# barlettacarmen/CrCNN

Hardware: AMD Instinct MI355X
Metric: encrypted images/sec (higher is better)
Workload: dtype u64

## Files before the change

### crcnn_amd/csrc/kernels_mfma.hip

```cpp
#include "kernels.h"
#include "limbred.h"
#include <algorithm>
#include <cstdlib>

typedef int v4i __attribute__((ext_vector_type(4)));
typedef int v16i __attribute__((ext_vector_type(16)));
typedef signed char i8;

#define NPL 7
#define TILE_B (NPL * 64 * 32)

struct MfmaArgs {
    const i8 *xl; const i8 *wl; u64 *ys; const ModParams *mods; const u64 *bias;
    int xcdmap;
    int mfast;
    i8 *xl_out; int lp2; unsigned zdp_out;
    int n, k, B, zdp, npos, yd, xs, ystr, yf, yo, P, F, Fp, zblks, ksteps, M, mtiles, ntiles;
    unsigned img_bytes; unsigned long long wslot_bytes; int ksteps_real;
    int flat, S, zdc; unsigned fplane;
    int sc_B;
    int acc0[8][13];
    u64 qinv[8];
};

__device__ __forceinline__ void limb_digits(u64 r, u64 q, int (&d)[NPL])
{
    long long v = r > (q >> 1) ? (long long)r - (long long)q : (long long)r;
#pragma unroll
    for (int l = 0; l < NPL; l++) { d[l] = (int)(signed char)(v & 0xff); v = (v - d[l]) >> 8; }
}

template <int NST>
__global__ void __launch_bounds__(256) __attribute__((amdgpu_waves_per_eu(1, 1))) mfma_mac_kernel(MfmaArgs a)
{
    extern __shared__ __attribute__((aligned(16))) i8 lds[];
    const int lane = threadIdx.x & 63, wave = __builtin_amdgcn_readfirstlane(threadIdx.x >> 6), wm = wave >> 1, wn = wave & 1;
    const int slots = a.n * a.k, per = a.mtiles * a.ntiles;
    int g = blockIdx.x, slot, tile;
    if ((slots & 7) == 0) { const int xcd = g & 7, r = g >> 3; slot = xcd * (slots >> 3) + r / per; tile = r % per; }
    else { slot = g / per; tile = g % per; }
    const int mt = a.mfast ? tile % a.mtiles : tile / a.ntiles, nt = a.mfast ? tile / a.mtiles : tile % a.ntiles;
    const int i = slot / a.n, s = slot % a.n;
    const int m0 = mt * 64, f0 = nt * 64;
    const ModParams m = a.mods[i];
    const u64 qinv = a.qinv[i];
    const i8 *xs = a.xl + (size_t)slot * a.B * a.img_bytes;
    const i8 *ws = a.wl + (size_t)slot * a.wslot_bytes + (size_t)f0 * 32;
    u32 src_off[7];
#pragma unroll
    for (int j = 0; j < 7; j++) {
        const int pc = wave + 4 * j;
        if (pc < 14) {
            const int c16 = pc * 64 + lane;
            const int plane = c16 >> 7, row = (c16 >> 1) & 63, half = c16 & 1;
            const int mm = min(m0 + row, a.M - 1);
            const int b = mm / (2 * a.P), p = (mm >> 1) % a.P, c = mm & 1;
            const int ox = p / a.yo, oy = p % a.yo;
            src_off[j] = a.npos == 1 ? (u32)(plane * a.zblks * (2 * a.B) + mm) * 32 + half * 16
                       : a.flat ? (u32)b * a.img_bytes + (u32)(plane * a.fplane + (c * a.npos + (ox * a.xs) * a.yd + oy * a.ystr) * a.zdc + half * 16)
                                : (u32)b * a.img_bytes + (u32)(plane * (a.npos * 2 * a.zdp) + (((ox * a.xs) * a.yd + oy * a.ystr) * 2 + c) * a.zdp + half * 16);
        } else src_off[j] = (u32)(((pc - 14) >> 1) * (a.Fp * 32) + ((pc - 14) & 1) * 1024 + lane * 16);
    }
    const int kreal = a.ksteps_real;
    auto issue = [&](int ks) {
        const int ka = min(ks, kreal - 1);
        const int tap = ka / a.zblks, zb = ka - tap * a.zblks;
        const int kx = tap / a.yf, ky = tap - kx * a.yf;
        const int fkx = ka / a.S;
        const u32 delta = a.npos == 1 ? (u32)zb * (2 * a.B) * 32 : a.flat ? (u32)(fkx * a.yd * a.zdc + (ka - fkx * a.S) * 32) : (u32)((kx * a.yd + ky) * 2 * a.zdp + zb * 32);
        i8 *dst = lds + (ks % NST) * (2 * TILE_B);
        const i8 *wt = ws + (size_t)ks * (NPL * a.Fp * 32);
#pragma unroll
        for (int j = 0; j < 7; j++) {
            const int pc = wave + 4 * j;
            const i8 *src = pc < 14 ? xs + src_off[j] + delta : wt + src_off[j];
            __builtin_amdgcn_global_load_lds((const __attribute__((address_space(1))) void *)src, (__attribute__((address_space(3))) void *)(dst + pc * 1024), 16, 0, 0);
        }
    };
    v4i acc[2][2][13];
#pragma unroll
    for (int rs = 0; rs < 2; rs++)
#pragma unroll
        for (int cs = 0; cs < 2; cs++)
#pragma unroll
            for (int d = 0; d < 13; d++) { const int b0 = a.acc0[i][d]; acc[rs][cs][d] = v4i{b0, b0, b0, b0}; }
    const int K = a.ksteps;
#pragma unroll
    for (int j = 0; j < NST - 2; j++) if (j < K) issue(j);
    const int kg = lane >> 4, r16 = lane & 15;
    const int fragA = (wm * 32 + r16) * 32 + (kg & 1) * 16, fragW = (wn * 32 + r16) * 32 + (kg & 1) * 16;
    for (int ks = 0; ks < K; ks += 2) {
        const int younger = min(NST - 4, K - 2 - ks);
        if (younger >= 1) __builtin_amdgcn_s_waitcnt(7 | (7 << 4) | (15 << 8));
        else __builtin_amdgcn_s_waitcnt(0 | (7 << 4) | (15 << 8));
        __syncthreads();
        __builtin_amdgcn_sched_barrier(0);
        if (ks + NST - 2 < K) { issue(ks + NST - 2); __builtin_amdgcn_sched_barrier(0); if (ks + NST - 1 < K) issue(ks + NST - 1); }
        __builtin_amdgcn_sched_barrier(0);
        const i8 *tA = lds + ((ks + (kg >> 1)) % NST) * (2 * TILE_B), *tW = tA + TILE_B;
        v4i w[2][NPL], av[2 * NPL];
        auto read_a = [&](int gi) { return *reinterpret_cast<const v4i *>(tA + (gi % NPL) * (64 * 32) + fragA + (gi / NPL) * (16 * 32)); };
#pragma unroll
        for (int cs = 0; cs < 2; cs++)
#pragma unroll
            for (int l = 0; l < NPL; l++) w[cs][l] = *reinterpret_cast<const v4i *>(tW + l * (64 * 32) + fragW + cs * (16 * 32));
        av[0] = read_a(0); av[1] = read_a(1);
        __builtin_amdgcn_sched_barrier(0);
#pragma unroll
        for (int gi = 0; gi < 2 * NPL; gi++) {
            const int rs = gi / NPL, l = gi % NPL;
#pragma unroll
            for (int cs = 0; cs < 2; cs++)
#pragma unroll
                for (int mm = 0; mm < NPL; mm++)
                    acc[rs][cs][l + mm] = __builtin_amdgcn_mfma_i32_16x16x64_i8(av[gi], w[cs][mm], acc[rs][cs][l + mm], 0, 0, 0);
            if (gi + 2 < 2 * NPL) av[gi + 2] = read_a(gi + 2);
            __builtin_amdgcn_sched_barrier(0);
        }
    }
    u64 *yslot = a.ys + (size_t)slot * a.B * a.F * (2 * a.P);
    const u32 P2 = 2 * a.P;
    const u32 RL = 64 * a.P;
    if (a.xl_out) __syncthreads();
#pragma unroll
    for (int rs = 0; rs < 2; rs++) {
        const u32 mbase = m0 + wm * 32 + rs * 16 + 4 * kg, bb = mbase / P2, rem = mbase - bb * P2;
#pragma unroll
        for (int cs = 0; cs < 2; cs++) {
            const int fl = wn * 32 + cs * 16 + r16, f = f0 + fl;
            const u64 bv = (a.bias && f < a.F) ? a.bias[((size_t)f * a.k + i) * a.n + s] : 0;
#pragma unroll
            for (int reg = 0; reg < 4; reg++) {
                int D[13];
#pragma unroll
                for (int d = 0; d < 13; d++) D[d] = acc[rs][cs][d][reg];
                u64 v = diag_reduce_w(D, m, qinv);
                if ((reg & 1) == 0) v = addmod(v, bv, m.q);
                if (a.xl_out) {
                    const u32 rt = wm * 32 + rs * 16 + 4 * kg + reg, bl = rt >> a.lp2, qq = rt & (P2 - 1);
                    const u64 dg = f < a.F ? balanced_digit_bytes(v, m.q) : 0;
                    i8 *sp = lds + (size_t)bl * (NPL * 2 * RL) + (qq & 1) * RL + fl * a.P + (qq >> 1);
#pragma unroll
                    for (int l = 0; l < NPL; l++) sp[(size_t)l * (2 * RL)] = (i8)(dg >> (8 * l));
                } else {
                    const u32 r = rem + reg, b = bb + (r >= P2) + (r >= 2 * P2);
                    if (mbase + reg < (u32)a.M && f < a.F) yslot[b * (u32)(a.F - 1) * P2 + (u32)f * P2 + mbase + reg] = v;
                }
                __builtin_amdgcn_sched_barrier(0);
            }
        }
    }
    if (a.xl_out) {
        __syncthreads();
        const u32 imgs = 64 >> a.lp2, b0 = (u32)m0 >> a.lp2, per_run = RL / 16, pieces = imgs * NPL * 2 * per_run;
        const u32 ch0 = (u32)f0 * a.P;
        for (u32 o = threadIdx.x; o < pieces; o += 256) {
            const u32 run = o / per_run, off = (o - run * per_run) * 16, bl = run / (NPL * 2), lc = run - bl * (NPL * 2);
            const u32 ch = ch0 + off;
            if (b0 + bl < (u32)a.B && ch < a.zdp_out)
                *reinterpret_cast<uint4 *>(a.xl_out + (size_t)slot * ((size_t)NPL * 2 * a.B * a.zdp_out)
                                           + ((size_t)((lc >> 1) * (a.zdp_out / 32) + (ch >> 5)) * (2 * a.B) + (b0 + bl) * 2 + (lc & 1)) * 32 + (ch & 31)) =
                    *reinterpret_cast<const uint4 *>(lds + (size_t)run * RL + off);
        }
    }
}

#define TILE_A (NPL * 64 * 32)
template <int NST, int MODE, bool SC = false>
__global__ void __launch_bounds__(256) __attribute__((amdgpu_waves_per_eu(2, 2))) mfma_mac2w_kernel(MfmaArgs a)
{
    extern __shared__ __attribute__((aligned(16))) i8 lds[];
    const int lane = threadIdx.x & 63, wave = __builtin_amdgcn_readfirstlane(threadIdx.x >> 6), wm = wave >> 1, wn = wave & 1;
    const int slots = a.n * a.k;
    const int fast = !SC && a.xcdmap ? (int)(blockIdx.x >> 3) : (int)blockIdx.x, slow = (int)blockIdx.y;
    const int slot = !SC && a.xcdmap ? (int)(blockIdx.x & 7) * (slots >> 3) + (int)blockIdx.z : (int)blockIdx.z;
    const int mt = SC || a.mfast ? fast : slow, nt = SC || a.mfast ? slow : fast;
    const int lgn = __builtin_ctz(a.n), i = SC ? slot : slot >> lgn, s = SC ? 0 : slot & (a.n - 1);
    const int m0 = mt * 64, f0 = nt * 32;
    if (f0 >= a.F) return;
    const ModParams m = a.mods[i];
    const u64 qinv = a.qinv[i];
    const i8 *xs = a.xl + (size_t)slot * a.B * a.img_bytes;
    const int kg = lane >> 4, r16 = lane & 15;
    const i8 *wlane = a.wl + (size_t)slot * a.wslot_bytes + (size_t)(f0 + wn * 16 + r16) * 32 + (kg & 1) * 16 + (size_t)(kg >> 1) * (NPL * a.Fp * 32);
    const int wplane = a.Fp * 32, wstep = NPL * a.Fp * 32;
    u32 src_off[4]; int pcs[4];
    {
        const int row = ((wave & 1) << 5) + (lane >> 1), half = lane & 1;
        const int mm = min(m0 + row, a.M - 1);
        const int b = mm / (2 * a.P), rem = mm - b * (2 * a.P), p = rem >> 1, c = rem & 1;
        const int ox = p / a.yo, oy = p - ox * a.yo;
        const u32 rowpart = MODE == 0 ? (u32)mm * 32 + half * 16
                          : MODE == 1 ? (u32)b * a.img_bytes + (u32)((c * a.npos + (ox * a.xs) * a.yd + oy * a.ystr) * a.zdc + half * 16)
                                   : (u32)b * a.img_bytes + (u32)((((ox * a.xs) * a.yd + oy * a.ystr) * 2 + c) * a.zdp + half * 16);
        const u32 pstride = MODE == 0 ? (u32)(a.zblks * (2 * a.B)) * 32 : MODE == 1 ? a.fplane : (u32)(a.npos * 2 * a.zdp);
#pragma unroll
        for (int j = 0; j < 4; j++) {
            pcs[j] = wave + 4 * j < 14 ? wave + 4 * j : wave + 8;
            src_off[j] = rowpart + (u32)(pcs[j] >> 1) * pstride;
        }
    }
    const int kreal = a.ksteps_real;
    int iss = 0, ibuf = 0, zb = 0, ky = 0, kx = 0;
    u32 delta = 0;
    auto issue_a = [&](int ks) {
        (void)ks;
        i8 *dst = lds + ibuf * TILE_A;
#pragma unroll
        for (int j = 0; j < 4; j++)
            __builtin_amdgcn_global_load_lds((const __attribute__((address_space(1))) void *)(xs + src_off[j] + delta), (__attribute__((address_space(3))) void *)(dst + pcs[j] * 1024), 16, 0, 0);
        iss++; ibuf = ibuf + 1 == NST ? 0 : ibuf + 1;
        if (iss < kreal) {
            if (MODE == 0) delta += (u32)(2 * a.B) * 32;
            else if (MODE == 1) { if (++zb == a.S) { zb = 0; kx++; } delta = (u32)(kx * a.yd * a.zdc + zb * 32); }
            else { if (++zb == a.zblks) { zb = 0; if (++ky == a.yf) { ky = 0; kx++; } } delta = (u32)((kx * a.yd + ky) * 2 * a.zdp + zb * 32); }
        }
    };
    auto load_w = [&](int ks, v4i (&w)[NPL]) {
        const i8 *pw = wlane + (size_t)ks * wstep;
#pragma unroll
        for (int l = 0; l < NPL; l++) w[l] = *reinterpret_cast<const v4i *>(pw + (size_t)l * wplane);
    };
    v4i acc[2][13];
#pragma unroll
    for (int rs = 0; rs < 2; rs++)
#pragma unroll
        for (int d = 0; d < 13; d++) { const int b0 = a.acc0[i][d]; acc[rs][d] = v4i{b0, b0, b0, b0}; }
    const int K = a.ksteps;
    const int fragA = (wm * 32 + r16) * 32 + (kg & 1) * 16;
    auto dstep = [&](int ks, v4i (&wuse)[NPL], v4i (&wload)[NPL]) {
        if (ks + 2 < K) __builtin_amdgcn_s_waitcnt(11 | (7 << 4) | (15 << 8));
        else __builtin_amdgcn_s_waitcnt(0 | (7 << 4) | (15 << 8));
        __syncthreads();
        __builtin_amdgcn_sched_barrier(0);
        if (ks + 3 < K) issue_a(ks + 3);
        __builtin_amdgcn_sched_barrier(0);
        if (ks + 4 < K) { load_w(ks + 4, wload); __builtin_amdgcn_sched_barrier(0); issue_a(ks + 4); }
        __builtin_amdgcn_sched_barrier(0);
        const i8 *tA = lds + ((ks + (kg >> 1)) % NST) * TILE_A;
        v4i av[2 * NPL];
        auto read_a = [&](int gi) { return *reinterpret_cast<const v4i *>(tA + (gi % NPL) * (64 * 32) + fragA + (gi / NPL) * (16 * 32)); };
        av[0] = read_a(0); av[1] = read_a(1); av[2] = read_a(2);
        __builtin_amdgcn_sched_barrier(0);
#pragma unroll
        for (int gi = 0; gi < 2 * NPL; gi++) {
            const int rs = gi / NPL, l = gi % NPL;
#pragma unroll
            for (int mm = 0; mm < NPL; mm++)
                acc[rs][l + mm] = __builtin_amdgcn_mfma_i32_16x16x64_i8(av[gi], wuse[mm], acc[rs][l + mm], 0, 0, 0);
            if (gi + 3 < 2 * NPL) av[gi + 3] = read_a(gi + 3);
            __builtin_amdgcn_sched_barrier(0);
        }
    };
    v4i w0[NPL], w1[NPL], w2[NPL];
    issue_a(0); if (1 < K) issue_a(1);
    __builtin_amdgcn_sched_barrier(0);
    load_w(0, w0);
    __builtin_amdgcn_sched_barrier(0);
    if (2 < K) { issue_a(2); __builtin_amdgcn_sched_barrier(0); load_w(2, w1); }
    __builtin_amdgcn_sched_barrier(0);
    for (int ks = 0; ks < K; ks += 6) {
        dstep(ks, w0, w2);
        if (ks + 2 < K) dstep(ks + 2, w1, w0);
        if (ks + 4 < K) dstep(ks + 4, w2, w1);
    }
    u64 *yslot = a.ys + (size_t)slot * a.B * a.F * (2 * a.P);
    const u32 P2 = 2 * a.P;
    const u32 RL = 32 * a.P;
    if (a.xl_out) __syncthreads();
    const int fl = wn * 16 + r16, f = f0 + fl;
    const u64 bv = (!SC && a.bias && f < a.F) ? a.bias[((size_t)f * a.k + i) * a.n + s] : 0;
    const u32 img_jump = (u32)(a.F - 1) * P2;
#pragma unroll
    for (int rs = 0; rs < 2; rs++) {
        const u32 mbase = m0 + wm * 32 + rs * 16 + 4 * kg, bb = mbase / P2, rem = mbase - bb * P2;
        const u32 idx0 = bb * img_jump + (u32)f * P2 + mbase;
#pragma unroll
        for (int reg = 0; reg < 4; reg++) {
            int D[13];
#pragma unroll
            for (int d = 0; d < 13; d++) D[d] = acc[rs][d][reg];
            u64 v = diag_reduce_w(D, m, qinv);
            if (SC) {
                if ((reg & 1) == 0 && a.bias && f < a.F && mbase + reg < (u32)a.M) {
                    const u32 r = rem + reg, e = bb + (r >= P2) + (r >= 2 * P2);
                    v = addmod(v, a.bias[((size_t)f * a.k + i) * a.n + e / (u32)a.sc_B], m.q);
                }
            } else if ((reg & 1) == 0) v = addmod(v, bv, m.q);
            if (a.xl_out) {
                const u32 rt = wm * 32 + rs * 16 + 4 * kg + reg, bl = rt >> a.lp2, qq = rt & (P2 - 1);
                const u64 dg = f < a.F ? balanced_digit_bytes(v, m.q) : 0;
                i8 *sp = lds + (size_t)bl * (NPL * 2 * RL) + (qq & 1) * RL + fl * a.P + (qq >> 1);
#pragma unroll
                for (int l = 0; l < NPL; l++) sp[(size_t)l * (2 * RL)] = (i8)(dg >> (8 * l));
            } else {
                const u32 r = rem + reg, jump = (r >= P2 ? img_jump : 0u) + (r >= 2 * P2 ? img_jump : 0u);
                if (mbase + reg < (u32)a.M && f < a.F) yslot[idx0 + reg + jump] = v;
            }
            __builtin_amdgcn_sched_barrier(0);
        }
    }
    if (a.xl_out) {
        __syncthreads();
        const u32 imgs = 64 >> a.lp2, b0 = (u32)m0 >> a.lp2, per_run = RL / 16, pieces = imgs * NPL * 2 * per_run;
        const u32 ch0 = (u32)f0 * a.P;
        for (u32 o = threadIdx.x; o < pieces; o += 256) {
            const u32 run = o / per_run, off = (o - run * per_run) * 16, bl = run / (NPL * 2), lc = run - bl * (NPL * 2);
            const u32 ch = ch0 + off;
            if (b0 + bl < (u32)a.B && ch < a.zdp_out)
                *reinterpret_cast<uint4 *>(a.xl_out + (size_t)slot * ((size_t)NPL * 2 * a.B * a.zdp_out)
                                           + ((size_t)((lc >> 1) * (a.zdp_out / 32) + (ch >> 5)) * (2 * a.B) + (b0 + bl) * 2 + (lc & 1)) * 32 + (ch & 31)) =
                    *reinterpret_cast<const uint4 *>(lds + (size_t)run * RL + off);
        }
    }
}

__global__ void __launch_bounds__(64) limb_pack_tensor_kernel(const u64 *x, i8 *xl, const ModParams *mods, int n, int k, int B, int zd, int zdp, int npos, int packed, int group,
                                                              int Btot, int b0, int flat_zdc, unsigned flat_img)
{
    const int sblocks = n / 64;
    const int sb = blockIdx.x % (sblocks * k), i = sb / sblocks, s = (sb % sblocks) * 64 + threadIdx.x;
    const int zblks = zdp / 32;
    const size_t items = (size_t)B * npos * 2 * zblks;
    const u64 q = mods[i].q;
    for (size_t r0 = (size_t)(blockIdx.x / (sblocks * k)) * group, u = 0; u < (size_t)group && r0 + u < items; u++) {
        size_t r = r0 + u;
        int zb, c, pos, b;
        if (npos == 1) { const size_t rows = (size_t)B * 2; zb = (int)(r / rows); r %= rows; c = (int)(r & 1); b = (int)(r >> 1); pos = 0; }
        else { zb = (int)(r % zblks); r /= zblks; c = (int)(r % 2); r /= 2; pos = (int)(r % npos); b = (int)(r / npos); }
        u32 pl[NPL][8];
#pragma unroll
        for (int l = 0; l < NPL; l++)
#pragma unroll
            for (int wv = 0; wv < 8; wv++) pl[l][wv] = 0;
#pragma unroll
        for (int z = 0; z < 32; z++) {
            const int zz = zb * 32 + z;
            if (zz < zd) {
                u64 v = x[((((size_t)b * zd * npos + (size_t)zz * npos + pos) * 2 + c) * k + i) * (size_t)n + s];
                if (packed) v = (v & 0xffffffffULL) | ((v >> 32) << 28);
                int d[NPL]; limb_digits(v, q, d);
#pragma unroll
                for (int l = 0; l < NPL; l++) pl[l][z >> 2] |= (u32)(d[l] & 0xff) << (8 * (z & 3));
            }
        }
        if (flat_zdc) {
            i8 *dstf = xl + (((size_t)i * n + s) * Btot + b0 + b) * (size_t)flat_img + ((size_t)c * npos + pos) * flat_zdc;
#pragma unroll
            for (int l = 0; l < NPL; l++) {
                u32 *o = reinterpret_cast<u32 *>(dstf + (size_t)l * 2 * npos * flat_zdc);
#pragma unroll
                for (int wv = 0; wv < 8; wv++) if (wv * 4 < flat_zdc) o[wv] = pl[l][wv];
            }
            continue;
        }
        i8 *dst = npos == 1 ? xl + ((size_t)i * n + s) * ((size_t)NPL * 2 * Btot * zdp) + ((size_t)zb * (2 * Btot) + (b0 + b) * 2 + c) * 32
                            : xl + (((size_t)i * n + s) * Btot + b0 + b) * ((size_t)NPL * npos * 2 * zdp) + ((size_t)pos * 2 + c) * zdp + zb * 32;
        const size_t plane_stride = npos == 1 ? (size_t)zblks * (2 * Btot) * 32 : (size_t)npos * 2 * zdp;
#pragma unroll
        for (int l = 0; l < NPL; l++) {
            uint4 *o = reinterpret_cast<uint4 *>(dst + (size_t)l * plane_stride);
            o[0] = make_uint4(pl[l][0], pl[l][1], pl[l][2], pl[l][3]); o[1] = make_uint4(pl[l][4], pl[l][5], pl[l][6], pl[l][7]);
        }
    }
}
#define TRG 4
#define TSL 32
__global__ void __launch_bounds__(256) limb_pack_dense_kernel(const u64 *x, i8 *xl, const ModParams *mods, int n, int k, int B, int zd, int zdp, int packed, int Btot, int b0, int scalar)
{
    __shared__ __attribute__((aligned(16))) i8 st[TSL * NPL * TRG * 32];
    const int sblocks = n / TSL, zblks = zdp / 32, rgs = (2 * B + TRG - 1) / TRG;
    const int sb = blockIdx.x % (sblocks * k), i = sb / sblocks, s0 = (sb % sblocks) * TSL;
    size_t r = blockIdx.x / (sblocks * k);
    const int rg = (int)(r % rgs), zb = (int)(r / rgs);
    const u64 q = mods[i].q;
    const int lane = threadIdx.x & (TSL - 1), qrow = (threadIdx.x >> 5) & (TRG - 1), h = threadIdx.x >> 7, row = rg * TRG + qrow;
    {
        u32 pl[NPL][4];
#pragma unroll
        for (int l = 0; l < NPL; l++)
#pragma unroll
            for (int wv = 0; wv < 4; wv++) pl[l][wv] = 0;
        if (row < 2 * B) {
            const int b = row >> 1, c = row & 1, z0 = zb * 32 + h * 16;
            const u64 *src = x + ((((size_t)b * zd + z0) * 2 + c) * k + i) * (size_t)n + s0 + lane;
#pragma unroll
            for (int z = 0; z < 16; z++)
                if (z0 + z < zd) {
                    u64 v = src[(size_t)z * 2 * k * n];
                    if (packed) v = (v & 0xffffffffULL) | ((v >> 32) << 28);
                    int d[NPL]; limb_digits(v, q, d);
#pragma unroll
                    for (int l = 0; l < NPL; l++) pl[l][z >> 2] |= (u32)(d[l] & 0xff) << (8 * (z & 3));
                }
        }
        i8 *sp = st + (size_t)lane * (NPL * TRG * 32) + qrow * 32 + h * 16;
#pragma unroll
        for (int l = 0; l < NPL; l++) *reinterpret_cast<uint4 *>(sp + l * (TRG * 32)) = make_uint4(pl[l][0], pl[l][1], pl[l][2], pl[l][3]);
    }
    __syncthreads();
    const int pieces_per_run = TRG * 2, rows_here = min(TRG, 2 * B - rg * TRG);
    const size_t plane_stride = (size_t)zblks * (2 * Btot) * 32, slot_stride = (size_t)NPL * plane_stride;
    for (int o = threadIdx.x; o < TSL * NPL * pieces_per_run; o += 256) {
        const int run = o / pieces_per_run, part = o - run * pieces_per_run, sl = run / NPL, l = run - sl * NPL;
        if ((part >> 1) >= rows_here) continue;
        i8 *dst = scalar ? xl + ((size_t)i * NPL + l) * (plane_stride * n) + (((size_t)zb * n + s0 + sl) * (2 * B) + rg * TRG) * 32 + part * 16
                         : xl + ((size_t)i * n + s0 + sl) * slot_stride + (size_t)l * plane_stride + ((size_t)zb * (2 * Btot) + (size_t)b0 * 2 + rg * TRG) * 32 + part * 16;
        *reinterpret_cast<uint4 *>(dst) = *reinterpret_cast<const uint4 *>(st + (size_t)run * (TRG * 32) + part * 16);
    }
}
#define WFG 4
#define WSL 32
__global__ void __launch_bounds__(256) limb_pack_weights_kernel(const u64 *w, i8 *wl, const ModParams *mods, int n, int k, int F, int Fz, int Fp, int zd, int zblks, int xf, int yf, int f0,
                                                                int flat_zdc, int S)
{
    __shared__ __attribute__((aligned(16))) i8 st[WSL * NPL * WFG * 32];
    const int sblocks = n / WSL, taps = xf * yf, steps = flat_zdc ? xf * S : taps * zblks;
    const int sb = blockIdx.x % (sblocks * k), i = sb / sblocks, s0 = (sb % sblocks) * WSL;
    size_t r = blockIdx.x / (sblocks * k);
    const int step = (int)(r % steps); const int fg = (int)(r / steps);
    const ModParams m = mods[i];
    const u64 R = barrett128(0, 1, m);
    const int lane = threadIdx.x & (WSL - 1), fq = (threadIdx.x >> 5) & (WFG - 1), h = threadIdx.x >> 7, f = fg * WFG + fq;
    {
        u32 pl[NPL][4];
#pragma unroll
        for (int l = 0; l < NPL; l++)
#pragma unroll
            for (int wv = 0; wv < 4; wv++) pl[l][wv] = 0;
        if (f < F) {
            int tap, ch, ky = 0, kx = 0;
            if (flat_zdc) { kx = step / S; const int j0 = (step - kx * S) * 32 + h * 16; ky = j0 / flat_zdc; ch = j0 - ky * flat_zdc; tap = kx * yf + ky; }
            else { tap = step / zblks; ch = (step - tap * zblks) * 32 + h * 16; }
#pragma unroll
            for (int z = 0; z < 16; z++) {
                if (ch < zd && (!flat_zdc || ky < yf)) {
                    const u64 v = mulmod(w[((((size_t)f * zd + ch) * taps + tap) * k + i) * (size_t)n + s0 + lane], R, m);
                    int d[NPL]; limb_digits(v, m.q, d);
#pragma unroll
                    for (int l = 0; l < NPL; l++) pl[l][z >> 2] |= (u32)(d[l] & 0xff) << (8 * (z & 3));
                }
                ch++;
                if (flat_zdc && ch == flat_zdc) { ch = 0; ky++; tap++; }
            }
        }
        i8 *sp = st + (size_t)lane * (NPL * WFG * 32) + fq * 32 + h * 16;
#pragma unroll
        for (int l = 0; l < NPL; l++) *reinterpret_cast<uint4 *>(sp + l * (WFG * 32)) = make_uint4(pl[l][0], pl[l][1], pl[l][2], pl[l][3]);
    }
    __syncthreads();
    const int pieces_per_run = WFG * 2, filters_here = min(WFG, Fz - fg * WFG);
    const size_t slot_stride = (size_t)((steps + 1) & ~1) * NPL * Fp * 32;
    for (int o = threadIdx.x; o < WSL * NPL * pieces_per_run; o += 256) {
        const int run = o / pieces_per_run, part = o - run * pieces_per_run, sl = run / NPL, l = run - sl * NPL;
        if ((part >> 1) >= filters_here) continue;
        i8 *dst = wl + ((size_t)i * n + s0 + sl) * slot_stride + (size_t)step * (NPL * Fp * 32) + (size_t)l * Fp * 32 + (size_t)(f0 + fg * WFG) * 32 + part * 16;
        *reinterpret_cast<uint4 *>(dst) = *reinterpret_cast<const uint4 *>(st + (size_t)run * (WFG * 32) + part * 16);
    }
}
__global__ void __launch_bounds__(256) slotmajor_to_rows_kernel(const u64 *ys, u64 *y, int n, int k, size_t rows, int pack_out)
{
    __shared__ u64 tile[64][65];
    const int sblocks = n / 64;
    const int sb = blockIdx.x % (sblocks * k), i = sb / sblocks, s0 = (sb % sblocks) * 64;
    const size_t e0 = (size_t)(blockIdx.x / (sblocks * k)) * 64;
    const int tx = threadIdx.x & 63, ty = threadIdx.x >> 6;
#pragma unroll
    for (int r = 0; r < 16; r++) {
        const int sl = r * 4 + ty;
        const size_t e = e0 + tx;
        tile[sl][tx] = e < rows ? ys[((size_t)i * n + s0 + sl) * rows + e] : 0;
    }
    __syncthreads();
#pragma unroll
    for (int r = 0; r < 16; r++) {
        const int el = r * 4 + ty;
        const size_t e = e0 + el;
        if (e < rows) { u64 v = tile[tx][el]; if (pack_out) v = (v & 0x0fffffffULL) | ((v >> 28) << 32); y[(e * k + i) * (size_t)n + s0 + tx] = v; }
    }
}
__global__ void __launch_bounds__(256) slotmajor_to_limb_kernel(const u64 *ys, i8 *xl, const ModParams *mods, int n, int B, int zd, int zdp, size_t total, int scalar)
{
    const size_t t = (size_t)blockIdx.x * blockDim.x + threadIdx.x;
    if (t >= total) return;
    const int zgs = zdp / 16;
    const int zg = (int)(t % zgs); size_t r = t / zgs; const int c = (int)(r % 2); r /= 2; const int b = (int)(r % B); const size_t slot = r / B;
    const u64 q = mods[slot / n].q;
    u32 pl[NPL][4];
#pragma unroll
    for (int l = 0; l < NPL; l++)
#pragma unroll
        for (int wv = 0; wv < 4; wv++) pl[l][wv] = 0;
    const u64 *src = ys + (slot * B + b) * (size_t)zd * 2 + c;
#pragma unroll
    for (int z = 0; z < 16; z++) {
        const int zz = zg * 16 + z;
        if (zz < zd) {
            int d[NPL]; limb_digits(src[(size_t)zz * 2], q, d);
#pragma unroll
            for (int l = 0; l < NPL; l++) pl[l][z >> 2] |= (u32)(d[l] & 0xff) << (8 * (z & 3));
        }
    }
    const size_t rows = scalar ? (size_t)n * 2 * B : (size_t)2 * B, row = (scalar ? (slot % n) * (size_t)(2 * B) : 0) + b * 2 + c, blk = scalar ? slot / n : slot;
    i8 *dst = xl + blk * ((size_t)NPL * rows * zdp) + ((size_t)(zg >> 1) * rows + row) * 32 + (zg & 1) * 16;
#pragma unroll
    for (int l = 0; l < NPL; l++) *reinterpret_cast<uint4 *>(dst + (size_t)l * (zdp / 32) * rows * 32) = make_uint4(pl[l][0], pl[l][1], pl[l][2], pl[l][3]);
}
__global__ void __launch_bounds__(256) scalar_pack_weights_kernel(const u64 *w, size_t wstride, i8 *wl, const ModParams *mods, int k, int F, int Fp, int zd, int zblks, int xf, int yf,
                                                                  int flat_zdc, int S, int steps, int steps_even)
{
    const size_t t = (size_t)blockIdx.x * blockDim.x + threadIdx.x;
    if (t >= (size_t)k * steps_even * Fp * 2) return;
    const int h = (int)(t & 1), f = (int)((t >> 1) % Fp);
    const int step = (int)((t >> 1) / Fp % steps_even), i = (int)((t >> 1) / Fp / steps_even), taps = xf * yf;
    const ModParams m = mods[i];
    const u64 R = barrett128(0, 1, m);
    u32 pl[NPL][4];
#pragma unroll
    for (int l = 0; l < NPL; l++)
#pragma unroll
        for (int wv = 0; wv < 4; wv++) pl[l][wv] = 0;
    if (f < F && step < steps) {
        int tap, ch, ky = 0, kx = 0;
        if (flat_zdc) { kx = step / S; const int j0 = (step - kx * S) * 32 + h * 16; ky = j0 / flat_zdc; ch = j0 - ky * flat_zdc; tap = kx * yf + ky; }
        else { tap = step / zblks; ch = (step - tap * zblks) * 32 + h * 16; }
#pragma unroll
        for (int z = 0; z < 16; z++) {
            if (ch < zd && (!flat_zdc || ky < yf)) {
                const u64 v = mulmod(w[((((size_t)f * zd + ch) * taps + tap) * k + i) * wstride], R, m);
                int d[NPL]; limb_digits(v, m.q, d);
#pragma unroll
                for (int l = 0; l < NPL; l++) pl[l][z >> 2] |= (u32)(d[l] & 0xff) << (8 * (z & 3));
            }
            ch++;
            if (flat_zdc && ch == flat_zdc) { ch = 0; ky++; tap++; }
        }
    }
    i8 *dst = wl + ((size_t)i * steps_even + step) * ((size_t)NPL * Fp * 32) + (size_t)f * 32 + h * 16;
#pragma unroll
    for (int l = 0; l < NPL; l++) *reinterpret_cast<uint4 *>(dst + (size_t)l * Fp * 32) = make_uint4(pl[l][0], pl[l][1], pl[l][2], pl[l][3]);
}
__global__ void __launch_bounds__(256) scalar_rows_constant_kernel(const u64 *w, size_t words, int n, int *flag)
{
    for (size_t t = (size_t)blockIdx.x * blockDim.x + threadIdx.x; t < words; t += (size_t)gridDim.x * blockDim.x)
        if (w[t] != w[t - (t & (size_t)(n - 1))]) *flag = 1;
}

static inline int round_up(int v, int m) { return (v + m - 1) / m * m; }
int k_limb_flat_zdc(int zd);
static void limb_tables(const crc_ctx *c, int T, int (*acc0)[13], u64 *qinv)
{
    for (int i = 0; i < c->k; i++) { limb_bias_table(c->tabs[i].m.q, T, acc0[i]); qinv[i] = inverse_mod_2_64(c->tabs[i].m.q); }
}

bool k_limb_supported(const crc_ctx *c, int T)
{
    if (c->n < 64 || T > 18000) return false;
    for (int i = 0; i < c->k; i++) if (c->tabs[i].m.bits > 55) return false;
    return true;
}
int k_limb_flat_zdc(int zd) { return zd < 32 ? round_up(zd, 4) : 0; }
int k_limb_steps(int zd, int xf, int yf) { const int zdc = k_limb_flat_zdc(zd); return zdc ? xf * ((yf * zdc + 31) / 32) : xf * yf * (round_up(zd, 32) / 32); }
static size_t limb_img_bytes(int zd, int npos) { const int zdc = k_limb_flat_zdc(zd); return zdc ? (size_t)round_up(NPL * 2 * npos * zdc, 16) : (size_t)NPL * npos * 2 * round_up(zd, 32); }
size_t k_limb_tensor_bytes(const crc_ctx *c, int B, int zd, int npos)
{
    if (npos == 1) return (size_t)c->n * c->k * B * NPL * 2 * round_up(zd, 32);
    return (size_t)c->n * c->k * B * limb_img_bytes(zd, npos) + 64;
}
size_t k_limb_weights_bytes(const crc_ctx *c, int nf, int zd, int xf, int yf) { return (size_t)c->n * c->k * round_up(k_limb_steps(zd, xf, yf), 2) * NPL * round_up(nf, 64) * 32; }
size_t k_limb_result_words(const crc_ctx *c, int B, int nf, int P) { return (size_t)c->n * c->k * B * nf * P * 2; }

int k_limb_pack_tensor(crc_ctx *c, const u64 *x, i8 *xl, int B, int zd, int npos, bool packed, hipStream_t st, int Btot, int b0, bool scalar)
{
    if (Btot <= 0) { Btot = B; b0 = 0; }
    if (b0 < 0 || b0 + B > Btot) return CRC_ERR_INVALID_ARGUMENT;
    if (npos > 1) scalar = false;
    if (scalar && (Btot != B || b0 != 0)) return CRC_ERR_INVALID_ARGUMENT;
    const int zdp = round_up(zd, 32);
    const int group = c->tune.limb_pack_group > 1 ? c->tune.limb_pack_group : (npos == 1 && (B * 2) % 4 == 0 ? 4 : 1);
    const size_t items = (size_t)B * npos * 2 * (zdp / 32);
    if (npos == 1 && (scalar || c->tune.limb_pack_group <= 1)) {
        const size_t blocks = (size_t)(c->n / TSL) * c->k * (zdp / 32) * ((2 * (size_t)B + TRG - 1) / TRG);
        if (blocks == 0) return CRC_OK;
        if (blocks > 0x7fffffffULL) return CRC_ERR_INVALID_ARGUMENT;
        hipLaunchKernelGGL(limb_pack_dense_kernel, dim3((unsigned)blocks), dim3(256), 0, st, x, xl, c->d_mods, c->n, c->k, B, zd, zdp, packed ? 1 : 0, Btot, b0, scalar ? 1 : 0);
        HIPCHK(hipGetLastError());
        return CRC_OK;
    }
    const size_t blocks = (size_t)(c->n / 64) * c->k * ((items + group - 1) / group);
    if (blocks == 0) return CRC_OK;
    if (blocks > 0x7fffffffULL) return CRC_ERR_INVALID_ARGUMENT;
    const int fz = npos > 1 ? k_limb_flat_zdc(zd) : 0;
    hipLaunchKernelGGL(limb_pack_tensor_kernel, dim3((unsigned)blocks), dim3(64), 0, st, x, xl, c->d_mods, c->n, c->k, B, zd, zdp, npos, packed ? 1 : 0, group, Btot, b0, fz,
                       (unsigned)limb_img_bytes(zd, npos));
    HIPCHK(hipGetLastError());
    return CRC_OK;
}
int k_limb_pack_weights(crc_ctx *c, const u64 *w, i8 *wl, int nf, int zd, int xf, int yf, hipStream_t st, int f0, int ft)
{
    if (ft < 0) ft = nf;
    if (f0 < 0 || ft < 1 || f0 + ft > nf) return CRC_ERR_INVALID_ARGUMENT;
    const int zblks = round_up(zd, 32) / 32, Fp = round_up(nf, 64), zdc = k_limb_flat_zdc(zd), S = zdc ? (yf * zdc + 31) / 32 : 0;
    const size_t step = (size_t)NPL * Fp * 32, steps = (size_t)k_limb_steps(zd, xf, yf), slot = (size_t)round_up((int)steps, 2) * step;
    if (f0 == 0 && (steps & 1)) HIPCHK(hipMemset2DAsync(wl + steps * step, slot, 0, step, (size_t)c->n * c->k, st));
    const int fz = f0 + ft == nf ? Fp - f0 : ft;
    const size_t blocks = (size_t)(c->n / WSL) * c->k * ((fz + WFG - 1) / WFG) * steps;
    if (blocks > 0x7fffffffULL) return CRC_ERR_INVALID_ARGUMENT;
    hipLaunchKernelGGL(limb_pack_weights_kernel, dim3((unsigned)blocks), dim3(256), 0, st, w, wl, c->d_mods, c->n, c->k, ft, fz, Fp, zd, zblks, xf, yf, f0, zdc, S);
    HIPCHK(hipGetLastError());
    return CRC_OK;
}
int k_limb_result_to_rows(crc_ctx *c, const u64 *ys, u64 *y, size_t rows, bool pack_out, hipStream_t st)
{
    const size_t blocks = (size_t)(c->n / 64) * c->k * ((rows + 63) / 64);
    if (blocks == 0) return CRC_OK;
// ... 110 lines not shown
```

### crcnn_amd/csrc/limbred.h

```cpp
#pragma once
#include "modarith.h"

CRC_HD u32 crc_alignbit(u32 hi, u32 lo, u32 sh)
{
#if defined(__HIP_DEVICE_COMPILE__)
    return __builtin_amdgcn_alignbit(hi, lo, sh);
#else
    return (u32)((((u64)hi << 32) | lo) >> sh);
#endif
}

CRC_HD u64 diag_reduce(const int (&D)[13], const ModParams &m, u64 qinv)
{
    typedef unsigned __int128 u128;
    const u128 s0 = ((u128)(((u64)(u32)D[12] << 32) | (u32)D[8]) << 64) | (((u64)(u32)D[4] << 32) | (u32)D[0]);
    const u128 s1 = ((u128)(u32)D[9] << 64) | (((u64)(u32)D[5] << 32) | (u32)D[1]);
    const u128 s2 = ((u128)(u32)D[10] << 64) | (((u64)(u32)D[6] << 32) | (u32)D[2]);
    const u128 s3 = ((u128)(u32)D[11] << 64) | (((u64)(u32)D[7] << 32) | (u32)D[3]);
    const u128 U = s0 + (s1 << 8) + (s2 << 16) + (s3 << 24);
    const u64 ulo = (u64)U, uhi = (u64)(U >> 64);
    const u64 mq = ulo * qinv;
    const u64 t = uhi - mulhi64(mq, m.q) + m.q;
    if (m.fold) {
        const u64 r = (t & (((u64)1 << m.bits) - 1)) + (u64)(u32)(t >> m.bits) * (u32)m.fold;
        return r >= m.q ? r - m.q : r;
    }
    return barrett128(t, 0, m);
}

CRC_HD u64 diag_reduce_w(const int (&D)[13], const ModParams &m, u64 qinv)
{
    typedef unsigned __int128 u128;
    const u32 a0 = (u32)D[1] << 8,  a1 = crc_alignbit((u32)D[5], (u32)D[1], 24), a2 = crc_alignbit((u32)D[9], (u32)D[5], 24),  a3 = (u32)D[9] >> 24;
    const u32 b0 = (u32)D[2] << 16, b1 = crc_alignbit((u32)D[6], (u32)D[2], 16), b2 = crc_alignbit((u32)D[10], (u32)D[6], 16), b3 = (u32)D[10] >> 16;
    const u32 c0 = (u32)D[3] << 24, c1 = crc_alignbit((u32)D[7], (u32)D[3], 8),  c2 = crc_alignbit((u32)D[11], (u32)D[7], 8),  c3 = (u32)D[11] >> 8;
    auto w128 = [](u32 w3, u32 w2, u32 w1, u32 w0) { return ((u128)(((u64)w3 << 32) | w2) << 64) | (((u64)w1 << 32) | w0); };
    const u128 U = w128((u32)D[12], (u32)D[8], (u32)D[4], (u32)D[0]) + w128(a3, a2, a1, a0) + w128(b3, b2, b1, b0) + w128(c3, c2, c1, c0);
    const u64 ulo = (u64)U, uhi = (u64)(U >> 64);
    const u64 mq = ulo * qinv;
    const u64 t = uhi - mulhi64(mq, m.q) + m.q;
    if (m.fold) {
        const u32 th = (u32)(t >> 32), sb = m.bits - 32;
        const u64 r = (((u64)(th & ((1u << sb) - 1)) << 32) | (u32)t) + (u64)(th >> sb) * (u32)m.fold;
        return r >= m.q ? r - m.q : r;
    }
    return barrett128(t, 0, m);
}

CRC_HD u64 diag_reduce_short(const int (&D)[13], u64 q, u64 qinv)
{
    u32 P[7];
    for (int j = 0; j < 6; j++) P[j] = (u32)D[2 * j] + ((u32)D[2 * j + 1] << 8);
    P[6] = (u32)D[12];
    const u32 o0 = P[1] << 16, o1 = (P[3] << 16) | (P[1] >> 16), o2 = (P[5] << 16) | (P[3] >> 16), o3 = P[5] >> 16;
    const u64 elo = ((u64)P[2] << 32) | P[0], ehi = ((u64)P[6] << 32) | P[4], olo = ((u64)o1 << 32) | o0, ohi = ((u64)o3 << 32) | o2;
    const u64 ulo = elo + olo, uhi = ehi + ohi + (ulo < elo);
    const u64 mq = ulo * qinv;
    const long long t = (long long)(uhi - mulhi64(mq, q));
    return (u64)(t + ((t >> 63) & (long long)q));
}

template <bool HAS_BIAS>
CRC_HD long long diag_reduce_short_centred(const int (&D)[13], u64 q, u64 qinv, long long bias_centred)
{
    typedef unsigned __int128 u128;
    u32 P[7];
    for (int j = 0; j < 6; j++) P[j] = (u32)D[2 * j] + ((u32)D[2 * j + 1] << 8);
    P[6] = (u32)D[12];
    const u128 E = ((u128)(((u64)P[6] << 32) | P[4]) << 64) | (((u64)P[2] << 32) | P[0]);
    const u128 O = ((u128)P[5] << 64) | (((u64)P[3] << 32) | P[1]);
    const u128 U = E + (O << 16);
    const u64 mq = (u64)U * qinv;
    long long t = (long long)((u64)(U >> 64) - mulhi64(mq, q));
    const long long h = (long long)(q >> 1);
    if (HAS_BIAS) t += bias_centred;
    t += t < -h ? (long long)q : 0;
    if (HAS_BIAS) t -= t > h ? (long long)q : 0;
    return t;
}
CRC_HD bool conv1_fold_ok(u64 q, u32 bits, u32 fold)
{
    typedef unsigned __int128 u128;
    if (bits < 53 || bits > 55 || fold == 0 || fold >= (1u << 26) || (((u64)1 << bits) - fold) != q) return false;
    const u128 uh_max = (((u128)0xC3) << 108) >> bits;
    return uh_max * fold + ((u128)1 << bits) < ((u128)1 << (bits + 32));
}
CRC_HD void diag_pack_words(const int (&D)[13], const u32 *PB, u32 (&u)[4])
{
    u32 P[7];
    for (int j = 0; j < 6; j++) P[j] = (u32)D[2 * j] + ((u32)D[2 * j + 1] << 8);
    P[6] = (u32)D[12];
    if (PB) for (int j = 0; j < 7; j++) P[j] += PB[j];
    const u32 o0 = P[1] << 16, o1 = crc_alignbit(P[3], P[1], 16), o2 = crc_alignbit(P[5], P[3], 16), o3 = P[5] >> 16;
    const u64 lo64 = (((u64)P[2] << 32) | P[0]) + (((u64)o1 << 32) | o0);
    const u64 hi64 = (((u64)P[6] << 32) | P[4]) + (((u64)o3 << 32) | o2) + (lo64 < (((u64)P[2] << 32) | P[0]));
    u[0] = (u32)lo64; u[1] = (u32)(lo64 >> 32); u[2] = (u32)hi64; u[3] = (u32)(hi64 >> 32);
}
CRC_HD long long fold_words_centred(u32 u0, u32 u1, u32 u2, u32 u3, u64 q, u32 bits, u32 fold, long long bias_centred)
{
    const u32 sb = bits - 32, m1 = (1u << sb) - 1;
    const u32 h0 = crc_alignbit(u2, u1, sb), h1 = crc_alignbit(u3, u2, sb);
    const u64 A = (u64)h0 * fold + (((u64)(u1 & m1) << 32) | u0);
    const u64 B = (u64)h1 * fold + (A >> 32);
    const u32 uh1 = crc_alignbit((u32)(B >> 32), (u32)B, sb);
    const u64 x2 = (u64)uh1 * fold + (((u64)((u32)B & m1) << 32) | (u32)A);
    u64 r = (u64)((u32)(x2 >> 32) >> sb) * fold + (((u64)((u32)(x2 >> 32) & m1) << 32) | (u32)x2);
    long long t = (long long)(r - q) + bias_centred;
    const long long h = (long long)(q >> 1);
    t += t < -h ? (long long)q : 0;
    t -= t > h ? (long long)q : 0;
    return t;
}
CRC_HD long long diag_fold_short_centred(const int (&D)[13], u64 q, u32 bits, u32 fold, long long bias_centred, const u32 *PB = nullptr)
{
    u32 u[4];
    diag_pack_words(D, PB, u);
    return fold_words_centred(u[0], u[1], u[2], u[3], q, bits, fold, bias_centred);
}
CRC_HD void diag7_pack_words(const int (&E)[7], const u32 *PB, u32 (&u)[3])
{
    u32 P[4];
    for (int j = 0; j < 3; j++) P[j] = (u32)E[2 * j] + ((u32)E[2 * j + 1] << 8);
    P[3] = (u32)E[6];
    if (PB) for (int j = 0; j < 4; j++) P[j] += PB[j];
    const u32 o0 = P[1] << 16, o1 = crc_alignbit(P[3], P[1], 16), o2 = P[3] >> 16;
    const u64 ev = ((u64)P[2] << 32) | P[0];
    const u64 lo64 = ev + (((u64)o1 << 32) | o0);
    u[0] = (u32)lo64; u[1] = (u32)(lo64 >> 32); u[2] = o2 + (lo64 < ev);
}
CRC_HD long long fold7_words_centred(u32 u0, u32 u1, u32 u2, u64 q, u32 bits, u32 fold, long long bias_centred)
{
    const u32 sb = bits - 32, m1 = (1u << sb) - 1;
    const u32 uh = crc_alignbit(u2, u1, sb);
    const u64 r = (u64)uh * fold + (((u64)(u1 & m1) << 32) | u0);
    long long t = (long long)(r - q) + bias_centred;
    const long long h = (long long)(q >> 1);
    t += t < -h ? (long long)q : 0;
    t -= t > h ? (long long)q : 0;
    return t;
}
CRC_HD long long diag7_fold_centred(const int (&E)[7], u64 q, u32 bits, u32 fold, long long bias_centred, const u32 *PB = nullptr)
{
    u32 u[3];
    diag7_pack_words(E, PB, u);
    return fold7_words_centred(u[0], u[1], u[2], q, bits, fold, bias_centred);
}
CRC_HD u64 centred_digit_bytes(long long cv) { return ((u64)cv + 0x0080808080808080ULL) ^ 0x0080808080808080ULL; }

CRC_HD u64 balanced_digit_bytes(u64 r, u64 q)
{
    const long long cv = r > (q >> 1) ? (long long)(r - q) : (long long)r;
    return ((u64)cv + 0x0080808080808080ULL) ^ 0x0080808080808080ULL;
}

CRC_HD u64 sum_reduce16(u64 s, u64 q)
{
    s -= s >= (q << 3) ? q << 3 : 0;
    s -= s >= (q << 2) ? q << 2 : 0;
    s -= s >= (q << 1) ? q << 1 : 0;
    s -= s >= q ? q : 0;
    return s;
}

inline u64 inverse_mod_2_64(u64 q) { u64 inv = q; for (int it = 0; it < 6; it++) inv *= 2 - q * inv; return inv; }

inline void bias_to_multiple(u64 q, long long (&B)[13])
{
    typedef unsigned __int128 u128;
    u128 K0 = 0;
    for (int d = 0; d < 13; d++) K0 += (u128)(u64)B[d] << (8 * d);
    const u64 rem = (u64)(K0 % q);
    long long delta = rem > q / 2 ? (long long)(q - rem) : -(long long)rem;
    for (int d = 0; d < 8 && delta; d++) { const long long dg = (long long)(signed char)(delta & 0xff); B[d] += dg; delta = (delta - dg) >> 8; }
}
inline void limb_bias_table(u64 q, int T, int (&out)[13])
{
    long long B[13];
    for (int d = 0; d < 13; d++) {
        const u64 bound = (u64)T * (u64)((d < 12 - d ? d : 12 - d) + 1) * 16384 + 256;
        u64 b = 1; while (b < bound) b <<= 1;
        B[d] = (long long)b;
    }
    bias_to_multiple(q, B);
    for (int d = 0; d < 13; d++) out[d] = (int)(u32)(u64)B[d];
}
inline void conv1_bias_table(u64 q, int (&out)[13])
{
    long long B[13];
    for (int d = 0; d < 13; d++) B[d] = d <= 10 ? 1 << 23 : d == 11 ? 1 << 21 : 1 << 19;
    bias_to_multiple(q, B);
    for (int d = 0; d < 13; d++) out[d] = (int)B[d];
}

inline void conv1_bias7_table(u64 q, int (&out)[7])
{
    typedef unsigned __int128 u128;
    long long B[7];
    u128 K0 = 0;
    for (int m = 0; m < 7; m++) { B[m] = 1 << 23; K0 += (u128)(u64)B[m] << (8 * m); }
    const u64 rem = (u64)(K0 % q);
    long long delta = rem > q / 2 ? (long long)(q - rem) : -(long long)rem;
    for (int m = 0; m < 7; m++) { const long long dg = (long long)(signed char)(delta & 0xff); B[m] += dg; delta = (delta - dg) >> 8; }
    for (int m = 0; m < 7; m++) out[m] = delta == 0 ? (int)B[m] : 0;
}
inline bool conv1_fold7_ok(u64 q, u32 bits, u32 fold)
{
    typedef unsigned __int128 u128;
    if (bits < 53 || bits > 55 || fold == 0 || fold >= (1u << 26) || (((u64)1 << bits) - fold) != q) return false;
    int B[7]; conv1_bias7_table(q, B);
    u128 umax = 0, k0 = 0;
    for (int m = 0; m < 7; m++) {
        if (B[m] <= 64 * 7 * 16384) return false;
        umax += (u128)(u64)(B[m] + 64 * 7 * 16384) << (8 * m); k0 += (u128)(u64)B[m] << (8 * m);
    }
    if (k0 % q != 0) return false;
    return (umax >> bits) * fold + ((u128)1 << bits) < (u128)2 * q;
}
```

Baseline: 779.3.

## Fuse centred reduction with digit split and pack LDS staging writes

When output limbs are produced and the modulus uses fold reduction, the epilogue now reduces accumulators directly to a centred representative, folding in bias, and extracts balanced digit bytes from it. This skips the separate canonical reduction, addmod and balanced conversion. Digit bytes from paired rows are combined with byte permutes into 16-bit LDS stores instead of individual byte stores. The LDS-to-global copy loop also swaps per-iteration divisions for incremental index updates. The cost is more code paths and reliance on centred_digit_bytes matching the old balanced encoding.

```diff
diff --git a/crcnn_amd/csrc/kernels_mfma.hip b/crcnn_amd/csrc/kernels_mfma.hip
--- a/crcnn_amd/csrc/kernels_mfma.hip
+++ b/crcnn_amd/csrc/kernels_mfma.hip
@@ -271,46 +271,98 @@
     const int fl = wn * 16 + r16, f = f0 + fl;
     const u64 bv = (!SC && a.bias && f < a.F) ? a.bias[((size_t)f * a.k + i) * a.n + s] : 0;
     const u32 img_jump = (u32)(a.F - 1) * P2;
-#pragma unroll
-    for (int rs = 0; rs < 2; rs++) {
-        const u32 mbase = m0 + wm * 32 + rs * 16 + 4 * kg, bb = mbase / P2, rem = mbase - bb * P2;
-        const u32 idx0 = bb * img_jump + (u32)f * P2 + mbase;
-#pragma unroll
-        for (int reg = 0; reg < 4; reg++) {
-            int D[13];
-#pragma unroll
-            for (int d = 0; d < 13; d++) D[d] = acc[rs][d][reg];
-            u64 v = diag_reduce_w(D, m, qinv);
-            if (SC) {
-                if ((reg & 1) == 0 && a.bias && f < a.F && mbase + reg < (u32)a.M) {
-                    const u32 r = rem + reg, e = bb + (r >= P2) + (r >= 2 * P2);
-                    v = addmod(v, a.bias[((size_t)f * a.k + i) * a.n + e / (u32)a.sc_B], m.q);
+    const bool centred = a.xl_out && m.fold;
+    if (centred) {
+        const long long bc = centred_rep(bv, m.q);
+        const u32 img_stage = NPL * 2 * RL, col = (u32)fl * a.P;
+#pragma unroll
+        for (int rs = 0; rs < 2; rs++) {
+            const u32 rt0 = wm * 32 + rs * 16 + 4 * kg;
+            u32 lo[4], hi[4];
+#pragma unroll
+            for (int reg = 0; reg < 4; reg++) {
+                int D[13];
+#pragma unroll
+                for (int d = 0; d < 13; d++) D[d] = acc[rs][d][reg];
+                long long cv;
+                if (reg & 1) cv = diag_reduce_w_centred<false>(D, m, qinv, 0);
+                else {
+                    long long brow = bc;
+                    if (SC) {
+                        brow = 0;
+                        if (a.bias && f < a.F && (u32)m0 + rt0 + reg < (u32)a.M) brow = centred_rep(a.bias[((size_t)f * a.k + i) * a.n + (((u32)m0 + rt0 + reg) >> a.lp2) / (u32)a.sc_B], m.q);
+                    }
+                    cv = diag_reduce_w_centred<true>(D, m, qinv, brow);
                 }
-            } else if ((reg & 1) == 0) v = addmod(v, bv, m.q);
-            if (a.xl_out) {
-                const u32 rt = wm * 32 + rs * 16 + 4 * kg + reg, bl = rt >> a.lp2, qq = rt & (P2 - 1);
-                const u64 dg = f < a.F ? balanced_digit_bytes(v, m.q) : 0;
-                i8 *sp = lds + (size_t)bl * (NPL * 2 * RL) + (qq & 1) * RL + fl * a.P + (qq >> 1);
-#pragma unroll
-                for (int l = 0; l < NPL; l++) sp[(size_t)l * (2 * RL)] = (i8)(dg >> (8 * l));
+                const u64 dg = f < a.F ? centred_digit_bytes(cv) : 0;
+                lo[reg] = (u32)dg; hi[reg] = (u32)(dg >> 32);
+                __builtin_amdgcn_sched_barrier(0);
+            }
+            if (a.lp2 >= 2) {
+                i8 *sp = lds + (rt0 >> a.lp2) * img_stage + col + ((rt0 & (P2 - 1)) >> 1);
+#pragma unroll
+                for (int c = 0; c < 2; c++, sp += RL) {
+                    const u32 p01 = __builtin_amdgcn_perm(lo[c + 2], lo[c], 0x05010400), p23 = __builtin_amdgcn_perm(lo[c + 2], lo[c], 0x07030602);
+                    const u32 p45 = __builtin_amdgcn_perm(hi[c + 2], hi[c], 0x05010400), p6 = __builtin_amdgcn_perm(hi[c + 2], hi[c], 0x0c0c0602);
+                    const u32 pr[4] = {p01, p23, p45, p6};
+#pragma unroll
+                    for (int l = 0; l < NPL; l++)
+                        *reinterpret_cast<unsigned short *>(sp + (size_t)l * (2 * RL)) = (unsigned short)(l & 1 ? pr[l >> 1] >> 16 : pr[l >> 1]);
+                }
             } else {
-                const u32 r = rem + reg, jump = (r >= P2 ? img_jump : 0u) + (r >= 2 * P2 ? img_jump : 0u);
-                if (mbase + reg < (u32)a.M && f < a.F) yslot[idx0 + reg + jump] = v;
+                i8 *sp = lds + (rt0 >> 1) * img_stage + col;
+#pragma unroll
+                for (int reg = 0; reg < 4; reg++) {
+                    i8 *sr = sp + (reg >> 1) * img_stage + (reg & 1) * RL;
+#pragma unroll
+                    for (int l = 0; l < NPL; l++) sr[(size_t)l * (2 * RL)] = (i8)((l < 4 ? lo[reg] : hi[reg]) >> (8 * (l & 3)));
+                }
             }
             __builtin_amdgcn_sched_barrier(0);
         }
+    } else {
+#pragma unroll
+        for (int rs = 0; rs < 2; rs++) {
+            const u32 mbase = m0 + wm * 32 + rs * 16 + 4 * kg, bb = mbase / P2, rem = mbase - bb * P2;
+            const u32 idx0 = bb * img_jump + (u32)f * P2 + mbase;
+#pragma unroll
+            for (int reg = 0; reg < 4; reg++) {
+                int D[13];
+#pragma unroll
+                for (int d = 0; d < 13; d++) D[d] = acc[rs][d][reg];
+                u64 v = diag_reduce_w(D, m, qinv);
+                if (SC) {
+                    if ((reg & 1) == 0 && a.bias && f < a.F && mbase + reg < (u32)a.M) {
+                        const u32 r = rem + reg, e = bb + (r >= P2) + (r >= 2 * P2);
+                        v = addmod(v, a.bias[((size_t)f * a.k + i) * a.n + e / (u32)a.sc_B], m.q);
+                    }
+                } else if ((reg & 1) == 0) v = addmod(v, bv, m.q);
+                if (a.xl_out) {
+                    const u32 rt = wm * 32 + rs * 16 + 4 * kg + reg, bl = rt >> a.lp2, qq = rt & (P2 - 1);
+                    const u64 dg = f < a.F ? balanced_digit_bytes(v, m.q) : 0;
+                    i8 *sp = lds + (size_t)bl * (NPL * 2 * RL) + (qq & 1) * RL + fl * a.P + (qq >> 1);
+#pragma unroll
+                    for (int l = 0; l < NPL; l++) sp[(size_t)l * (2 * RL)] = (i8)(dg >> (8 * l));
+                } else {
+                    const u32 r = rem + reg, jump = (r >= P2 ? img_jump : 0u) + (r >= 2 * P2 ? img_jump : 0u);
+                    if (mbase + reg < (u32)a.M && f < a.F) yslot[idx0 + reg + jump] = v;
+                }
+                __builtin_amdgcn_sched_barrier(0);
+            }
+        }
     }
     if (a.xl_out) {
         __syncthreads();
-        const u32 imgs = 64 >> a.lp2, b0 = (u32)m0 >> a.lp2, per_run = RL / 16, pieces = imgs * NPL * 2 * per_run;
-        const u32 ch0 = (u32)f0 * a.P;
-        for (u32 o = threadIdx.x; o < pieces; o += 256) {
-            const u32 run = o / per_run, off = (o - run * per_run) * 16, bl = run / (NPL * 2), lc = run - bl * (NPL * 2);
-            const u32 ch = ch0 + off;
+        const u32 b0 = (u32)m0 >> a.lp2, ch = (u32)f0 * a.P + ((threadIdx.x & (P2 - 1)) << 4), zb_out = a.zdp_out >> 5;
+        const u32 drun = 256u >> a.lp2, dbl = drun / (NPL * 2), dlc = drun - dbl * (NPL * 2);
+        u32 run = threadIdx.x >> a.lp2, bl = run / (NPL * 2), lc = run - bl * (NPL * 2);
+        i8 *yo = a.xl_out + (size_t)slot * ((size_t)NPL * 2 * a.B * a.zdp_out) + (ch & 31);
+        const i8 *sp = lds + ((threadIdx.x & (P2 - 1)) << 4);
+        for (u32 o = threadIdx.x; o < 64u * NPL * 2; o += 256) {
             if (b0 + bl < (u32)a.B && ch < a.zdp_out)
-                *reinterpret_cast<uint4 *>(a.xl_out + (size_t)slot * ((size_t)NPL * 2 * a.B * a.zdp_out)
-                                           + ((size_t)((lc >> 1) * (a.zdp_out / 32) + (ch >> 5)) * (2 * a.B) + (b0 + bl) * 2 + (lc & 1)) * 32 + (ch & 31)) =
-                    *reinterpret_cast<const uint4 *>(lds + (size_t)run * RL + off);
+                *reinterpret_cast<uint4 *>(yo + (size_t)(((lc >> 1) * zb_out + (ch >> 5)) * (u32)(2 * a.B) + (b0 + bl) * 2 + (lc & 1)) * 32) = *reinterpret_cast<const uint4 *>(sp + run * RL);
+            run += drun; bl += dbl; lc += dlc;
+            if (lc >= NPL * 2) { lc -= NPL * 2; bl++; }
         }
     }
 }
diff --git a/crcnn_amd/csrc/limbred.h b/crcnn_amd/csrc/limbred.h
--- a/crcnn_amd/csrc/limbred.h
+++ b/crcnn_amd/csrc/limbred.h
@@ -28,7 +28,7 @@
     return barrett128(t, 0, m);
 }
 
-CRC_HD u64 diag_reduce_w(const int (&D)[13], const ModParams &m, u64 qinv)
+CRC_HD u64 diag_mont_w(const int (&D)[13], u64 q, u64 qinv)
 {
     typedef unsigned __int128 u128;
     const u32 a0 = (u32)D[1] << 8,  a1 = crc_alignbit((u32)D[5], (u32)D[1], 24), a2 = crc_alignbit((u32)D[9], (u32)D[5], 24),  a3 = (u32)D[9] >> 24;
@@ -38,14 +38,33 @@
     const u128 U = w128((u32)D[12], (u32)D[8], (u32)D[4], (u32)D[0]) + w128(a3, a2, a1, a0) + w128(b3, b2, b1, b0) + w128(c3, c2, c1, c0);
     const u64 ulo = (u64)U, uhi = (u64)(U >> 64);
     const u64 mq = ulo * qinv;
-    const u64 t = uhi - mulhi64(mq, m.q) + m.q;
+    return uhi - mulhi64(mq, q) + q;
+}
+CRC_HD u64 fold_upper_word(u64 t, const ModParams &m)
+{
+    const u32 th = (u32)(t >> 32), sb = m.bits - 32;
+    return (((u64)(th & ((1u << sb) - 1)) << 32) | (u32)t) + (u64)(th >> sb) * (u32)m.fold;
+}
+CRC_HD u64 diag_reduce_w(const int (&D)[13], const ModParams &m, u64 qinv)
+{
+    const u64 t = diag_mont_w(D, m.q, qinv);
     if (m.fold) {
-        const u32 th = (u32)(t >> 32), sb = m.bits - 32;
-        const u64 r = (((u64)(th & ((1u << sb) - 1)) << 32) | (u32)t) + (u64)(th >> sb) * (u32)m.fold;
+        const u64 r = fold_upper_word(t, m);
         return r >= m.q ? r - m.q : r;
     }
     return barrett128(t, 0, m);
 }
+template <bool HAS_BIAS>
+CRC_HD long long diag_reduce_w_centred(const int (&D)[13], const ModParams &m, u64 qinv, long long bias_centred)
+{
+    long long t = (long long)(fold_upper_word(diag_mont_w(D, m.q, qinv), m) - m.q);
+    const long long h = (long long)(m.q >> 1);
+    if (HAS_BIAS) t += bias_centred;
+    t += t < -h ? (long long)m.q : 0;
+    if (HAS_BIAS) t -= t > h ? (long long)m.q : 0;
+    return t;
+}
+CRC_HD long long centred_rep(u64 r, u64 q) { return r > (q >> 1) ? (long long)(r - q) : (long long)r; }
 
 CRC_HD u64 diag_reduce_short(const int (&D)[13], u64 q, u64 qinv)
 {
```

Measured after the change: 795.8 (median of 6 runs). 1.02x the previous value.
